# Funatiq/cuclark

Measured on AMD Instinct MI355X. Metric: Mreads/sec (10M x 150bp, k=31), higher is better.
Workload: dtype u64

## Files before the change

cuclark_amd/csrc/mic_kernels.hip:

```cpp
#include "mic_internal.h"
#include "mic_device.h"
#include "mic_ksketch.h"

#include <stdlib.h>

#ifndef MIC_EXP
#define MIC_EXP 0
#endif
#ifndef MIC_FUNNEL64
#define MIC_FUNNEL64 1
#endif
#ifndef MIC_X
#define MIC_X 0
#endif

namespace {

__device__ __forceinline__ uint4 load_slot_quarter(const uint4* p) {
  typedef unsigned int u4 __attribute__((ext_vector_type(4)));
  u4 t = __builtin_nontemporal_load((const u4*)p);
  return make_uint4(t.x, t.y, t.z, t.w);
}

__device__ __forceinline__ uint64_t kmer_from_dwords(uint32_t d0, uint32_t d1, uint32_t d2, int nt_in_dword, int k) {
  const int s = 2 * nt_in_dword;
  uint64_t a = ((uint64_t)d0 << 32) | d1;
#if MIC_FUNNEL64
  uint64_t x = (a << s) | ((uint64_t)d2 >> (32 - s));
#else
  uint64_t x = s ? ((a << s) | (uint64_t)(d2 >> (32 - s))) : a;
#endif
  return x >> (64 - 2 * k);
}


struct ReadAhead { uint32_t pp, pe, hdr, w; };

__device__ __forceinline__ void ahead_ptr(const MicQueryArgs& a, uint32_t r, ReadAhead& x) {
  if (r < a.n_reads) { x.pp = a.reads_ptr[r]; x.pe = a.reads_ptr[r + 1]; } else { x.pp = 0; x.pe = 0; }
}

__device__ __forceinline__ void ahead_window(const uint16_t* __restrict__ cont, uint32_t r, uint32_t n_reads, int lane,
                                             ReadAhead& x) {
  x.hdr = 0; x.w = 0;
  if (r < n_reads) {
    const uint32_t pp = __builtin_amdgcn_readfirstlane(x.pp);
    x.hdr = cont[pp];
    if (lane < 10) x.w = ((uint32_t)cont[pp + 1 + 2 * lane] << 16) | cont[pp + 2 + 2 * lane];
  }
}

__device__ __forceinline__ uint32_t window_word(const uint16_t* __restrict__ cont, uint32_t first, uint32_t cend,
                                                uint32_t base, int lane, bool use_ahead, const ReadAhead& x) {
  uint32_t w = 0;
  const uint32_t ci = first + base / 8 + 2 * lane;
  if (use_ahead) w = x.w;
  else if (lane < 10) w = ((ci < cend ? (uint32_t)cont[ci] : 0u) << 16) | (ci + 1 < cend ? (uint32_t)cont[ci + 1] : 0u);
  if (lane >= 10 || ci >= cend) w &= 0x0000FFFFu;
  if (lane >= 10 || ci + 1 >= cend) w &= 0xFFFF0000u;
  return w;
}

__device__ __forceinline__ uint32_t window_word_w(const uint16_t* __restrict__ cont, uint32_t first, uint32_t cend,
                                                  uint32_t base, int lane, bool use_ahead, uint32_t ahead_w) {
  uint32_t w = 0;
  const uint32_t ci = first + base / 8 + 2 * lane;
  if (use_ahead) w = ahead_w;
  else if (lane < 10) w = ((ci < cend ? (uint32_t)cont[ci] : 0u) << 16) | (ci + 1 < cend ? (uint32_t)cont[ci + 1] : 0u);
  if (lane >= 10 || ci >= cend) w &= 0x0000FFFFu;
  if (lane >= 10 || ci + 1 >= cend) w &= 0xFFFF0000u;
  return w;
}

struct Probe {
  uint32_t slot;
  uint32_t qlo, qhi;
};

template <bool KEY64>
__device__ __forceinline__ Probe make_probe(const MicTable& t, uint64_t kmer, bool active) {
  uint64_t c = canonical(kmer, t.k);
  uint64_t q = mic_div(c, t.div);
  uint64_t rem = c - q * t.div.d;
  Probe p;
  bool ok = active && rem >= t.shard_start && rem < t.shard_end;
  if (!KEY64) ok = ok && (q >> 32) == 0;
  p.slot = ok ? (uint32_t)(rem - t.shard_start) : 0xFFFFFFFFu;
// ... 245 lines not shown
  if (cover < w) step(w - cover);
}

__device__ __forceinline__ void sliding_min2(uint32_t& a0, uint32_t& a1, int w, int lane) {
  auto step = [&](int s) {
    const int src = (lane + s) & 63;
    const bool wrap = lane + s >= 64;
    uint32_t x0 = bperm(src, a0), x1 = bperm(src, a1);
    uint32_t n0 = wrap ? x1 : x0, n1 = wrap ? 0xFFFFFFFFu : x1;
    a0 = n0 < a0 ? n0 : a0; a1 = n1 < a1 ? n1 : a1;
  };
  int cover = 1;
  while (2 * cover <= w) { step(cover); cover *= 2; }
  if (cover < w) step(w - cover);
}

__device__ __forceinline__ uint32_t row_prefix_min(uint32_t t) {
  uint32_t x;
  x = (uint32_t)__builtin_amdgcn_update_dpp(-1, (int)t, 0x111, 0xF, 0xF, false); t = x < t ? x : t;
  x = (uint32_t)__builtin_amdgcn_update_dpp(-1, (int)t, 0x112, 0xF, 0xF, false); t = x < t ? x : t;
  x = (uint32_t)__builtin_amdgcn_update_dpp(-1, (int)t, 0x114, 0xF, 0xF, false); t = x < t ? x : t;
  x = (uint32_t)__builtin_amdgcn_update_dpp(-1, (int)t, 0x118, 0xF, 0xF, false); t = x < t ? x : t;
  return t;
}

__device__ __forceinline__ uint32_t row_suffix_min(uint32_t t) {
  uint32_t x;
  x = (uint32_t)__builtin_amdgcn_update_dpp(-1, (int)t, 0x101, 0xF, 0xF, false); t = x < t ? x : t;
  x = (uint32_t)__builtin_amdgcn_update_dpp(-1, (int)t, 0x102, 0xF, 0xF, false); t = x < t ? x : t;
  x = (uint32_t)__builtin_amdgcn_update_dpp(-1, (int)t, 0x104, 0xF, 0xF, false); t = x < t ? x : t;
  x = (uint32_t)__builtin_amdgcn_update_dpp(-1, (int)t, 0x108, 0xF, 0xF, false); t = x < t ? x : t;
  asm("" : "+v"(t));
  return t;
}

template <int BANKS>
__device__ __forceinline__ uint32_t with_row_in_front(uint32_t P) {
  const uint32_t f = (uint32_t)__builtin_amdgcn_update_dpp(-1, (int)P, 0x142, 0xE, BANKS, false);
  return f < P ? f : P;
}
__device__ __forceinline__ void sliding_min_rows(uint32_t& a0, uint32_t& a1, uint32_t a2, int W, int lane, int lane_inv) {
  const uint32_t P0 = row_prefix_min(a0), P1 = row_prefix_min(a1), P2 = row_prefix_min(a2);
  if (W > 16 && ((W - 16) & 3) == 0) {
    const uint32_t S0 = row_suffix_min(a0), S1 = row_suffix_min(a1);
    const int s = W - 16, bm = (1 << (s >> 2)) - 1;
    uint32_t Q0, Q1, Q2;
    switch (bm) {
      case 1: Q0 = with_row_in_front<1>(P0); Q1 = with_row_in_front<1>(P1); Q2 = with_row_in_front<1>(P2); break;
      case 3: Q0 = with_row_in_front<3>(P0); Q1 = with_row_in_front<3>(P1); Q2 = with_row_in_front<3>(P2); break;
      case 7: Q0 = with_row_in_front<7>(P0); Q1 = with_row_in_front<7>(P1); Q2 = with_row_in_front<7>(P2); break;
      default: Q0 = with_row_in_front<15>(P0); Q1 = with_row_in_front<15>(P1); Q2 = with_row_in_front<15>(P2); break;
    }
    const uint32_t f0 = __builtin_amdgcn_readlane(P0, 63), f1 = __builtin_amdgcn_readlane(P1, 63);
    const bool head = lane < s;
    const uint32_t h1 = f0 < Q1 ? f0 : Q1, h2 = f1 < Q2 ? f1 : Q2;
    Q1 = head ? h1 : Q1; Q2 = head ? h2 : Q2;
    const int at = (lane_inv << 2) + ((W - 1) << 2);
    const uint32_t z0 = (uint32_t)__builtin_amdgcn_ds_bpermute(at, (int)Q0), z1 = (uint32_t)__builtin_amdgcn_ds_bpermute(at, (int)Q1),
                   z2 = (uint32_t)__builtin_amdgcn_ds_bpermute(at, (int)Q2);
    const bool wz = lane >= 65 - W;
    const uint32_t v0 = wz ? z1 : z0, v1 = wz ? z2 : z1;
    a0 = v0 < S0 ? v0 : S0; a1 = v1 < S1 ? v1 : S1;
    return;
  }
  const uint32_t S0 = row_suffix_min(a0), S1 = row_suffix_min(a1), S2 = row_suffix_min(a2);
  const int at = lane_inv << 2;
  const uint32_t x0 = (uint32_t)__builtin_amdgcn_ds_bpermute(at + 60, (int)P0), x1 = (uint32_t)__builtin_amdgcn_ds_bpermute(at + 60, (int)P1),
                 x2 = (uint32_t)__builtin_amdgcn_ds_bpermute(at + 60, (int)P2);
  const bool wr = lane >= 49;
  const uint32_t n0 = wr ? x1 : x0, n1 = wr ? x2 : x1;
  uint32_t M0 = n0 < S0 ? n0 : S0, M1 = n1 < S1 ? n1 : S1;
  if (W > 16) {
    const uint32_t M2 = x2 < S2 ? x2 : S2;
    const int sh = (W - 16) << 2;
    const uint32_t y0 = (uint32_t)__builtin_amdgcn_ds_bpermute(at + sh, (int)M0), y1 = (uint32_t)__builtin_amdgcn_ds_bpermute(at + sh, (int)M1),
                   y2 = (uint32_t)__builtin_amdgcn_ds_bpermute(at + sh, (int)M2);
    const bool wy = lane >= 80 - W;
    const uint32_t v0 = wy ? y1 : y0, v1 = wy ? y2 : y1;
    M0 = v0 < M0 ? v0 : M0; M1 = v1 < M1 ? v1 : M1;
  }
  a0 = M0; a1 = M1;
}

template <bool CANON>
__device__ __forceinline__ void sampled_positions(uint32_t wd, int ln, int lane_inv, int k, int m, bool past, uint32_t& qa0, uint32_t& qa1) {
  const int w = k - m + 1, t = s_tlen(k, m), W = k - t + 1;
  const uint32_t pb = (uint32_t)lane_inv & 31u;
  uint32_t a0, a1, a2 = 0xFFFFFFFFu;
  if (t <= 16) {
    const int s1 = lane_inv - 1;
    const int ad = (s1 >> 4) << 2;
    const uint32_t tsh = 30u - 2u * (uint32_t)(s1 & 15);
    auto tkey = [&](int h) {
      const uint32_t W0 = (uint32_t)__builtin_amdgcn_ds_bpermute(ad + 16 * h, (int)wd), W1 = (uint32_t)__builtin_amdgcn_ds_bpermute(ad + 16 * h + 4, (int)wd);
      uint32_t tv = __builtin_amdgcn_alignbit(W0, W1, tsh) >> (32 - 2 * t);
      if (CANON) { const uint32_t tr = revcomp_bits32(tv, t); tv = tr < tv ? tr : tv; }
      return ((t <= 12 ? s_torder24(tv) : s_torder(tv)) & ~31u) | pb;
    };
    a0 = tkey(0); a1 = tkey(1);
    if (past) a2 = tkey(2);
  } else {
    auto tkey = [&](int h) {
      const int idx = 4 * h + (lane_inv >> 4);
      const uint32_t d0 = bperm(idx, wd), d1 = bperm(idx + 1, wd), d2 = bperm(idx + 2, wd);
      uint64_t tv = kmer_from_dwords(d0, d1, d2, lane_inv & 15, t);
      if (CANON) { const uint64_t tr = revcomp_bits(tv, t); tv = tr < tv ? tr : tv; }
      return (s_torder(tv) & ~31u) | pb;
    };
    a0 = tkey(0); a1 = tkey(1);
    if (past) a2 = tkey(2);
  }
  if (W >= 16) sliding_min_rows(a0, a1, a2, W, ln, lane_inv);
  else sliding_min3(a0, a1, a2, W, ln);
  uint32_t d0 = (a0 - pb) & 31u, d1 = (a1 - pb) & 31u;
  if (W == 2 * w) { const uint32_t e0 = d0 - (uint32_t)w, e1 = d1 - (uint32_t)w; d0 = e0 < d0 ? e0 : d0; d1 = e1 < d1 ? e1 : d1; }
  else if (W != w) {
    const uint32_t rcp = (1024u + (uint32_t)w - 1u) / (uint32_t)w;
    d0 -= (uint32_t)w * ((d0 * rcp) >> 10); d1 -= (uint32_t)w * ((d1 * rcp) >> 10);
  }
  qa0 = (uint32_t)lane_inv + d0; qa1 = 64u + (uint32_t)lane_inv + d1;
}

template <bool CANON>
__device__ __forceinline__ void sampled_positions3(uint32_t wd, int lane_inv, uint32_t n_act, uint32_t& p0, uint32_t& s0, uint32_t& s1, uint32_t& s2,
                                                    uint32_t& q0, uint32_t& q1, uint32_t& q2) {
  const int at = lane_inv << 2;
  const int ad = f3_dword(lane_inv) << 2;
  const uint32_t tsh = f3_shift(lane_inv);
  p0 = 3u * (uint32_t)lane_inv;
  const uint32_t np0 = 0u - p0;
  const uint32_t W0 = (uint32_t)__builtin_amdgcn_ds_bpermute(ad, (int)wd), W1 = (uint32_t)__builtin_amdgcn_ds_bpermute(ad + 4, (int)wd);
  const uint32_t X = __builtin_amdgcn_alignbit(W0, W1, tsh);
  uint32_t t0 = f3_tmer(X, 0), t1 = f3_tmer(X, 1), t2 = f3_tmer(X, 2);
  if (CANON) {
    const uint32_t br = __builtin_bitreverse32(X);
    const uint32_t Y = swap_comp_pairs(br >> 1, br << 1);
    t0 = f3_min(t0, f3_tmer_rc(Y, 0)); t1 = f3_min(t1, f3_tmer_rc(Y, 1)); t2 = f3_min(t2, f3_tmer_rc(Y, 2));
  }
  auto key = [](uint32_t tv, uint32_t pos) { return (uint32_t)__builtin_amdgcn_bitop3_b32(s_torder24(tv), pos, 31u, 0xD8); };
  const uint32_t k0 = key(t0, p0), k1 = key(t1, p0 + 1u), k2 = key(t2, p0 + 2u);
  const uint32_t T = f3_min3(k0, k1, k2), e12 = f3_min(k1, k2), e01 = f3_min(k0, k1);
  const uint32_t x1 = (uint32_t)__builtin_amdgcn_ds_bpermute(at + 4, (int)T);
  const uint32_t m2 = f3_min(T, x1);
  const uint32_t y = (uint32_t)__builtin_amdgcn_ds_bpermute(at + 8, (int)m2);
  const uint32_t m4 = f3_min(m2, y);
  const uint32_t z = (uint32_t)__builtin_amdgcn_ds_bpermute(at + 16, (int)m4);
  const uint32_t k0n = (uint32_t)__builtin_amdgcn_ds_bpermute(at + 32, (int)k0), e01n = (uint32_t)__builtin_amdgcn_ds_bpermute(at + 32, (int)e01);
  uint32_t r0, r1, r2;
  f3_combine(k2, e12, m4, x1, y, z, k0n, e01n, r0, r1, r2);
  auto sampled = [&](uint32_t r, uint32_t j) {
    const uint32_t d = (r + np0 - j) & 31u, e = d - (uint32_t)F3_WM;
    return f3_min(d, e) + p0 + j;
  };
  const int nv = (int)(n_act + np0);
  s0 = sampled(r0, 0u); s1 = sampled(r1, 1u); s2 = sampled(r2, 2u);
  q0 = nv > 0 ? s0 : ~0u; q1 = nv > 1 ? s1 : ~0u; q2 = nv > 2 ? s2 : ~0u;
}

#ifndef MIC_SPEC
#define MIC_SPEC 1
#endif
#ifndef MIC_M_WPB
#define MIC_M_WPB 4
#endif
template <int KK, int MM>
__global__ void __launch_bounds__(64 * MIC_M_WPB, 32 / MIC_M_WPB) query_kernel_m(const MicQueryArgs a) {
  __shared__ uint4 s_stage[MIC_M_WPB][MIC_RMAX * MIC_MSTRIDE + (MIC_RMAX / 8 - 1) * MIC_M_SKEW];
  __shared__ uint32_t s_run[MIC_M_WPB][MIC_RMAX];
  __shared__ uint32_t s_ahead[MIC_M_WPB][2][64];
  const int lane = threadIdx.x & 63;
  const int wv = __builtin_amdgcn_readfirstlane(threadIdx.x >> 6);
  uint4* stage = s_stage[wv];
  uint32_t* runslot = s_run[wv];
  const uint32_t wave0 = __builtin_amdgcn_readfirstlane(blockIdx.x * MIC_M_WPB + wv);
  const uint32_t n_waves = gridDim.x * MIC_M_WPB;
  const MicTable& t = a.t;
  const int k = KK ? KK : t.k, m = MM ? MM : t.m, w = k - m + 1;
  const uint4* __restrict__ slots = t.slots;
  const uint16_t* __restrict__ cont = a.cont;
  auto below = [](uint64_t mask) { return (uint32_t)__builtin_amdgcn_mbcnt_hi((uint32_t)(mask >> 32), __builtin_amdgcn_mbcnt_lo((uint32_t)mask, 0u)); };

  uint32_t* ahead0 = s_ahead[wv][0];
  uint32_t* ahead1 = s_ahead[wv][1];
  auto ahead_issue = [&](uint32_t* entry, uint32_t pp_w, uint32_t r_ptr) {
    const uint64_t abase = ((uint64_t)(cont + pp_w)) & ~3ULL;
    const uint32_t rr = r_ptr < a.n_reads ? r_ptr : a.n_reads - 1;
    const uint64_t pbase = (uint64_t)(a.reads_ptr + rr) - 48;
    uint32_t lv = (uint32_t)lane;
    asm volatile("" : "+v"(lv));
    const uint32_t li = lv < 14 ? lv : 0u;
    const uint64_t addr = (li < 12 ? abase : pbase) + 4 * li;
    __builtin_amdgcn_global_load_lds((const __attribute__((address_space(1))) void*)addr,
                                     (__attribute__((address_space(3))) void*)entry, 4, 0, 0);
  };
  auto ahead_take = [&](const uint32_t* entry, uint32_t pp_w, uint32_t& hdr, uint32_t& wword, uint32_t& npp, uint32_t& npe) {
    const uint32_t raw = entry[lane];
    npp = __builtin_amdgcn_readlane(raw, 12); npe = __builtin_amdgcn_readlane(raw, 13);
    const bool odd = (((uint64_t)(cont + pp_w)) >> 1) & 1;
    const uint32_t up = (uint32_t)__builtin_amdgcn_update_dpp(0, (int)raw, 0x101, 0xF, 0xF, true);
    const uint32_t first = __builtin_amdgcn_readfirstlane(raw);
    hdr = odd ? first >> 16 : first & 0xFFFFu;
    wword = odd ? ((up << 16) | (up >> 16)) : ((raw & 0xFFFF0000u) | (up & 0xFFFFu));
  };
  uint32_t cur_pp, cur_pe, cur_hdr, cur_w;
  uint32_t n_pp, n_pe;
  uint32_t ahead_sel;
  {
    const uint32_t r0 = wave0 < a.n_reads ? wave0 : a.n_reads - 1;
    cur_pp = __builtin_amdgcn_readfirstlane(a.reads_ptr[r0]); cur_pe = __builtin_amdgcn_readfirstlane(a.reads_ptr[r0 + 1]);
    ahead_issue(ahead0, cur_pp, wave0 + n_waves);
    asm volatile("s_waitcnt vmcnt(0)" ::: "memory");
    __builtin_amdgcn_wave_barrier();
    ahead_take(ahead0, cur_pp, cur_hdr, cur_w, n_pp, n_pe);
    ahead_issue(ahead1, n_pp, wave0 + 2 * n_waves);
    ahead_sel = 1;
  }
  for (uint32_t r = wave0; r < a.n_reads; r += n_waves) {
    uint32_t pp = cur_pp;
    const uint32_t pe = cur_pe;
    RowAcc acc; acc.label1 = 0; acc.count = 0;
    uint32_t n_ent = 0, overflow = 0, total = 0;
    bool first_part = true;

    while (pp < pe) {
      const uint32_t plen = __builtin_amdgcn_readfirstlane(first_part ? cur_hdr : (uint32_t)cont[pp]);
      const bool ahead_ok = first_part;
      first_part = false;
      if (plen == 0) break;
      const uint32_t first = pp + 1;
      pp = first + (plen + 7) / 8;
      if (plen < (uint32_t)k) continue;
      const uint32_t nk = plen - k + 1;
      const uint32_t cend = pp;
      for (uint32_t base = 0; base < nk; base += 128) {
        const uint32_t wd = window_word_w(cont, first, cend, base, lane, ahead_ok && base == 0, cur_w);
        uint64_t c[2]; bool act[2]; uint32_t hk0, hk1, hk2;
        const bool past = nk - base > (uint32_t)(129 - w);
        const bool tail_path = w <= 16;
        uint32_t tail = 0xFFFFFFFFu;
// ... 436 lines not shown
    const uint32_t l1 = __builtin_amdgcn_readlane(lab1, __builtin_ctzll(mm));
    const bool mine = lab1 == l1;
    mm &= ~wballot(mine);
    const uint32_t c = mine ? cnt : 0u;
    uint32_t sum = 0;
    {
      uint32_t v = c;
      v += (uint32_t)__builtin_amdgcn_update_dpp(0, (int)v, 0x111, 0xF, 0xF, true);
      v += (uint32_t)__builtin_amdgcn_update_dpp(0, (int)v, 0x112, 0xF, 0xF, true);
      v += (uint32_t)__builtin_amdgcn_update_dpp(0, (int)v, 0x114, 0xF, 0xF, true);
      v += (uint32_t)__builtin_amdgcn_update_dpp(0, (int)v, 0x118, 0xF, 0xF, true);
      sum = __builtin_amdgcn_readlane(v, 15) + __builtin_amdgcn_readlane(v, 31);
    }
    total += sum;
    row_add(acc, n_ent, overflow, l1, sum, lane);
  }
}

template <int KK, int MM, bool FWD, bool PART>
__global__ void __launch_bounds__(64 * MIC_M_WPB, 32 / MIC_M_WPB) query_kernel_r(const MicQueryArgs a) {
  __shared__ uint4 s_stage[MIC_M_WPB][MIC_RMAX * MIC_MSTRIDE + (MIC_RMAX / 8 - 1) * MIC_R_SKEW];
  __shared__ uint16_t s_rec[MIC_M_WPB][132];
  __shared__ uint32_t s_ahead[MIC_M_WPB][2][64];
  __shared__ uint32_t s_part[PART ? MIC_M_WPB : 1][2];
  const int lane = threadIdx.x & 63;
  const int wv = __builtin_amdgcn_readfirstlane(threadIdx.x >> 6);
  uint4* stage = s_stage[wv];
  uint16_t* rec = s_rec[wv];
  const uint32_t wave0 = __builtin_amdgcn_readfirstlane(blockIdx.x * MIC_M_WPB + wv);
  const uint32_t n_waves = gridDim.x * MIC_M_WPB;
  const MicTable& t = a.t;
  if (PART) { if (lane == 0) { s_part[wv][0] = t.slot_lo; s_part[wv][1] = t.slot_cnt; } __builtin_amdgcn_wave_barrier(); }
  const int k = KK ? KK : t.k, m = MM ? MM : t.m, ctx = k - m;
  const uint4* __restrict__ slots = t.slots;
  const uint16_t* __restrict__ cont = a.cont;
  auto below = [](uint64_t mask) { return (uint32_t)__builtin_amdgcn_mbcnt_hi((uint32_t)(mask >> 32), __builtin_amdgcn_mbcnt_lo((uint32_t)mask, 0u)); };

  uint32_t* ahead0 = s_ahead[wv][0];
  uint32_t* ahead1 = s_ahead[wv][1];
  auto ahead_issue = [&](uint32_t* entry, uint32_t pp_w, uint32_t r_ptr) {
    const uint64_t abase = ((uint64_t)(cont + pp_w)) & ~3ULL;
    const uint32_t rr = r_ptr < a.n_reads ? r_ptr : a.n_reads - 1;
    const uint64_t pbase = (uint64_t)(a.reads_ptr + rr) - 48;
    int ln = lane;
    asm volatile("" : "+v"(ln));
    if (ln < 12)
      __builtin_amdgcn_global_load_lds((const __attribute__((address_space(1))) void*)((const uint32_t*)abase + lane),
                                       (__attribute__((address_space(3))) void*)entry, 4, 0, 0);
    uint64_t pb = pbase + 48;
    asm volatile("" : "+s"(pb));
    if (ln < 2)
      __builtin_amdgcn_global_load_lds((const __attribute__((address_space(1))) void*)((const uint32_t*)pb + lane),
                                       (__attribute__((address_space(3))) void*)(entry + 12), 4, 0, 0);
  };
  auto ahead_take = [&](const uint32_t* entry, uint32_t pp_w, uint32_t& hdr, uint32_t& npp, uint32_t& npe) {
    const uint32_t raw = entry[lane];
    npp = __builtin_amdgcn_readlane(raw, 12); npe = __builtin_amdgcn_readlane(raw, 13);
    const bool odd = (((uint64_t)(cont + pp_w)) >> 1) & 1;
    const uint32_t first = __builtin_amdgcn_readfirstlane(raw);
    hdr = odd ? first >> 16 : first & 0xFFFFu;
  };
  auto ahead_word = [&](const uint32_t* entry, uint32_t pp_w) {
    const uint32_t raw = entry[lane];
    const bool odd = (((uint64_t)(cont + pp_w)) >> 1) & 1;
    const uint32_t up = (uint32_t)__builtin_amdgcn_update_dpp(0, (int)raw, 0x101, 0xF, 0xF, true);
    return __builtin_amdgcn_perm(up, raw, odd ? 0x05040706u : 0x03020504u);
  };
  uint32_t cur_pp, cur_pe, cur_hdr, n_pp, n_pe, ahead_sel;
  {
    const uint32_t r0 = wave0 < a.n_reads ? wave0 : a.n_reads - 1;
    cur_pp = __builtin_amdgcn_readfirstlane(a.reads_ptr[r0]); cur_pe = __builtin_amdgcn_readfirstlane(a.reads_ptr[r0 + 1]);
    ahead_issue(ahead0, cur_pp, wave0 + n_waves);
    asm volatile("s_waitcnt vmcnt(0)" ::: "memory");
    __builtin_amdgcn_wave_barrier();
    ahead_take(ahead0, cur_pp, cur_hdr, n_pp, n_pe);
    ahead_issue(ahead1, n_pp, wave0 + 2 * n_waves);
    ahead_sel = 1;
  }
  constexpr bool PIPE = KK != 0 && (MIC_R_PIPE >= 2 || (MIC_R_PIPE == 1 && FWD));
  struct Round {
    uint32_t G0, G1, G2, cur;
    int jmax, jmin, remaining;
  };
  auto front = [&](const uint32_t first, const uint32_t cend, const uint32_t base, const uint32_t nk, const bool use_ahead, uint32_t& wd_out) __attribute__((always_inline)) -> uint32_t {
    int ln = lane;
    asm volatile("" : "+v"(ln));
    const uint32_t wd = use_ahead ? ahead_word(ahead_sel ? ahead0 : ahead1, cur_pp)
                                  : window_word_w(cont, first, cend, base, ln, false, 0u);
    wd_out = wd;
    const uint32_t n_act = nk - base < 128u ? nk - base : 128u;
    if constexpr (KK == F3_K && MM == F3_M) {
      uint32_t p0, s0, s1, s2, q0, q1, q2;
      sampled_positions3<!FWD>(wd, lane, n_act, p0, s0, s1, s2, q0, q1, q2);
      const uint32_t pv = (uint32_t)__builtin_amdgcn_update_dpp(-1, (int)q2, 0x138, 0xF, 0xF, false);
      const bool f0 = q0 != pv, f1 = q1 != q0, f2 = q2 != q1;
      const uint64_t b0 = wballot(f0), b1 = wballot(f1), b2 = wballot(f2);
      const uint32_t R = __popcll(b0) + __popcll(b1) + __popcll(b2) - 1u;
      uint32_t c = __builtin_amdgcn_mbcnt_hi((uint32_t)(b0 >> 32), __builtin_amdgcn_mbcnt_lo((uint32_t)b0, 0u));
      c = __builtin_amdgcn_mbcnt_hi((uint32_t)(b1 >> 32), __builtin_amdgcn_mbcnt_lo((uint32_t)b1, c));
      c = __builtin_amdgcn_mbcnt_hi((uint32_t)(b2 >> 32), __builtin_amdgcn_mbcnt_lo((uint32_t)b2, c));
      __builtin_amdgcn_wave_barrier();
      const uint32_t c1 = c + (f0 ? 1u : 0u), c2 = c1 + (f1 ? 1u : 0u);
      if (f0) rec[c] = f3_record(s0, p0);
      if (f1) rec[c1] = f3_record(s1, p0 + 1u);
      if (f2) rec[c2] = f3_record(s2, p0 + 2u);
      __builtin_amdgcn_wave_barrier();
      return R;
    }
    const bool past = n_act + (uint32_t)(k - s_tlen(k, m)) >= 129u;
    uint32_t qa0, qa1;
    sampled_positions<!FWD>(wd, ln, lane, k, m, past, qa0, qa1);
    qa0 = (uint32_t)lane < n_act ? qa0 : 0xFFu;
    qa1 = 64u + (uint32_t)lane < n_act ? qa1 : 0xFFu;
    const uint32_t last0 = __builtin_amdgcn_readlane(qa0, 63);
    uint32_t p0 = (uint32_t)__builtin_amdgcn_update_dpp(-1, (int)qa0, 0x138, 0xF, 0xF, false);
    uint32_t p1 = (uint32_t)__builtin_amdgcn_update_dpp((int)last0, (int)qa1, 0x138, 0xF, 0xF, false);
    const bool f0 = qa0 != p0, f1 = qa1 != p1;
    const uint64_t b0 = wballot(f0), b1 = wballot(f1);
    const uint32_t R0 = __popcll(b0), R = R0 + __popcll(b1) - (n_act < 128u ? 1u : 0u);
    __builtin_amdgcn_wave_barrier();
    if (f0) rec[below(b0)] = (uint16_t)(qa0 | ((uint32_t)lane << 8));
    if (f1) rec[R0 + below(b1)] = (uint16_t)(qa1 | ((64u + (uint32_t)lane) << 8));
    if (__builtin_expect(n_act == 128u, 0)) {
      asm volatile("" ::: "memory");
      if (ln == 0) rec[R] = (uint16_t)(128u << 8);
    }
    __builtin_amdgcn_wave_barrier();
    return R;
  };
  const uint32_t xsh = (64u - 2u * (uint32_t)k) & 31u;
  auto region_x = [&](uint32_t A0, uint32_t A1, uint32_t& lo, uint32_t& hi) {
    if (k > 16) {
      lo = __builtin_amdgcn_alignbit(A0, A1, xsh) & (m >= 16 ? 0xFFFFFFFFu : (1u << ((2 * m) & 31)) - 1u);
      hi = m > 16 ? (A0 >> xsh) & ((1u << ((2 * m - 32) & 31)) - 1u) : 0u;
    } else {
      const uint64_t x = ((((uint64_t)A0 << 32) | A1) << (2 * ctx)) >> (64 - 2 * m);
      lo = (uint32_t)x; hi = (uint32_t)(x >> 32);
    }
  };
  auto setup = [&](const uint32_t wd, const uint32_t rbase, const uint32_t R, Round& L, uint32_t& nrun_out) __attribute__((always_inline)) {
    const uint32_t nrun = R - rbase < MIC_RMAX ? R - rbase : MIC_RMAX;
    nrun_out = nrun;
    const bool vr = (uint32_t)lane < nrun;
    const uint32_t ri = vr ? rbase + (uint32_t)lane : 0u;
    const uint32_t rc0 = rec[ri], rc1 = rec[ri + 1];
    const int qa = (int)(rc0 & 255u), i0 = (int)(rc0 >> 8);
    const int n = (int)(rc1 >> 8) - i0;
    const int s1 = qa - ctx - 1;
    const int D = s1 >> 4;
    const uint32_t tsh = 30u - 2u * (uint32_t)(s1 & 15);
    const int a0 = D << 2;
    const uint32_t W0 = (uint32_t)__builtin_amdgcn_ds_bpermute(a0, (int)wd), W1 = (uint32_t)__builtin_amdgcn_ds_bpermute(a0 + 4, (int)wd),
                   W2 = (uint32_t)__builtin_amdgcn_ds_bpermute(a0 + 8, (int)wd), W3 = (uint32_t)__builtin_amdgcn_ds_bpermute(a0 + 12, (int)wd);
    uint32_t G0 = __builtin_amdgcn_alignbit(W0, W1, tsh), G1 = __builtin_amdgcn_alignbit(W1, W2, tsh), G2 = __builtin_amdgcn_alignbit(W2, W3, tsh);
    uint32_t key, xhi;
    region_x(G0, G1, key, xhi);
    bool rev = false;
    if (!FWD) {
      const uint32_t sh = 96u - 2u * (uint32_t)(k + ctx);
      const uint32_t r0 = __builtin_bitreverse32(G2), r1 = __builtin_bitreverse32(G1), r2 = __builtin_bitreverse32(G0);
      uint32_t q0, q1, q2;
      if (KK != 0 && sh != 0) {
        q0 = swap_comp_pairs(__builtin_amdgcn_alignbit(r0, r1, 33u - sh), __builtin_amdgcn_alignbit(r0, r1, 31u - sh));
        q1 = swap_comp_pairs(__builtin_amdgcn_alignbit(r1, r2, 33u - sh), __builtin_amdgcn_alignbit(r1, r2, 31u - sh));
        q2 = swap_comp_pairs(r2 << (sh - 1u), r2 << (sh + 1u));
      } else {
        q0 = sh ? __builtin_amdgcn_alignbit(r0, r1, 32u - sh) : r0;
        q1 = sh ? __builtin_amdgcn_alignbit(r1, r2, 32u - sh) : r1;
        q2 = r2 << sh;
        q0 = swap_comp_pairs(q0 >> 1, q0 << 1); q1 = swap_comp_pairs(q1 >> 1, q1 << 1); q2 = swap_comp_pairs(q2 >> 1, q2 << 1);
      }
      uint32_t kr, hr;
      region_x(q0, q1, kr, hr);
      rev = hr < xhi || (hr == xhi && kr < key);
      G0 = rev ? q0 : G0; G1 = rev ? q1 : G1; G2 = rev ? q2 : G2;
      key = rev ? kr : key; xhi = rev ? hr : xhi;
    }
    const int jmaxf = qa - i0, jminf = jmaxf - n + 1;
    const int jmax = rev ? ctx - jminf : jmaxf, jmin = rev ? ctx - jmaxf : jminf;
    uint32_t cur = vr ? sslot_of_x32(key, xhi, (uint32_t)t.n_main) : 0xFFFFFFFFu;
    bool mine = vr;
    if (PART) {
      mine = vr && cur - s_part[wv][0] < s_part[wv][1];
      cur = mine ? cur : 0xFFFFFFFFu;
    }
    L.G0 = G0; L.G1 = G1; L.G2 = G2; L.cur = cur;
    L.jmax = jmax; L.jmin = jmin; L.remaining = mine ? n : 0;
  };
  auto issue = [&](const uint32_t cur, const uint32_t nrun) __attribute__((always_inline)) {
    uint32_t sidx[MIC_RMAX / 8];
    int ln = lane;
    asm volatile("" : "+v"(ln));
    __builtin_amdgcn_wave_barrier();
    if (ln < MIC_RMAX) ((uint32_t*)stage)[lane] = cur;
    __builtin_amdgcn_wave_barrier();
    uint32_t so = (uint32_t)(uintptr_t)(__attribute__((address_space(3))) void*)stage;
    asm volatile("" : "+s"(so));
#pragma unroll
    for (int i = 0; i < MIC_RMAX / 8; ++i) sidx[i] = ((const uint32_t*)stage)[8 * i + (lane >> 3)];
#pragma unroll
    for (int i = 0; i < MIC_RMAX / 8; ++i) {
      if (8u * i >= nrun) break;
      if (sidx[i] != 0xFFFFFFFFu)
        __builtin_amdgcn_global_load_lds((const __attribute__((address_space(1))) void*)(slots + (uint64_t)sidx[i] * 8 + (lane & 7)),
                                         (__attribute__((address_space(3))) void*)(uintptr_t)(so + 16u * (64 + MIC_R_SKEW) * (uint32_t)i), 16, 0, 0);
    }
  };
  auto consume = [&](Round& L, RowAcc& acc, uint32_t& n_ent, uint32_t& overflow, uint32_t& total, uint32_t& cg) __attribute__((always_inline)) {
    const uint32_t G0 = L.G0, G1 = L.G1, G2 = L.G2;
    uint32_t key, xhi_;
    region_x(G0, G1, key, xhi_);
    const int jmax = L.jmax, jmin = L.jmin;
    uint32_t cur = L.cur;
    int remaining = L.remaining;
    bool again = false;
    do {
      if (again) issue(cur, MIC_RMAX);
      again = true;
      asm volatile("s_waitcnt vmcnt(0)" ::: "memory");
      __builtin_amdgcn_wave_barrier();
      const bool vl = cur != 0xFFFFFFFFu;
      const uint32_t* q = (const uint32_t*)(stage + (vl ? staged_at((uint32_t)lane) : 0));
      const uint4 ka = *(const uint4*)q;
      const uint2 kb = *(const uint2*)(q + 4);
      uint32_t e = (ka.x < key) + (ka.y < key) + (ka.z < key) + (ka.w < key) + (kb.x < key) + (kb.y < key);
      const uint32_t mz = q[30];
      bool more = vl && e < 6;
      e = e < 5 ? e : 5;
      for (;;) {
// ... 17 lines not shown
#if !(MIC_X & 1)
        remaining = (same && mineq && (pl >> 16) == 0) ? MIC_R_CROWDED : remaining;
#endif
        const uint32_t lab_new = (pl & 0xFFFFu) + 1u;
        tally_counts(hits ? lab_new : 0u, hits, acc, n_ent, overflow, total, lane);
        remaining -= (int)hits;
        more = same && remaining > 0 && e < 5;
        e += more ? 1u : 0u;
        if (!wballot(more)) break;
      }
      const bool nx = vl && remaining > 0 && (mz & MIC_S_NEXT);
      cur = 0xFFFFFFFFu;
      if (wballot(nx)) { if (nx && q[5] <= key) cur = q[31]; }
    } while (wballot(cur != 0xFFFFFFFFu));
    if (!(MIC_X & 2) && __builtin_expect(wballot(remaining <= MIC_R_CROWDED) != 0, 0)) {
      const bool crowded = remaining <= MIC_R_CROWDED;
      const uint32_t n_c = (uint32_t)__popcll(wballot(crowded));
      uint64_t kpv = (uint64_t)__builtin_amdgcn_kernarg_segment_ptr();
      asm volatile("" : "+v"(kpv));
      const MicQueryArgs* kv = (const MicQueryArgs*)kpv;
      uint32_t* cw = kv->crowd;
      uint32_t* itb = kv->crowd_items;
      const uint32_t icap = kv->crowd_item_cap;
      uint32_t ib = 0xFFFFFFFFu;
      if (cw != nullptr && cg != MIC_CG_DENSE) {
        uint32_t v = 0;
        if (lane == 0) v = atomicAdd(&cw[1], n_c);
        ib = __builtin_amdgcn_readfirstlane(v);
      }
      asm volatile("" : "+v"(ib));
      const bool room = ib <= icap && n_c <= icap - ib;
      if (crowded && room) {
        uint32_t* it = itb + 8 * ((size_t)ib + below(wballot(crowded)));
        it[0] = G0; it[1] = G1; it[2] = G2; it[3] = (uint32_t)jmin | ((uint32_t)jmax << 8);
        it[4] = cg;
      }
      cg = __builtin_amdgcn_readfirstlane(room ? (ib | ((n_c - 1u) << 27)) : MIC_CG_DENSE);
    }
  };
  auto finish = [&](const RowAcc& acc, uint32_t n_ent, uint32_t total, uint32_t overflow, uint32_t r, const uint32_t cg) __attribute__((always_inline)) {
    uint32_t spilled = 0;
    if (!(MIC_X & 4) && __builtin_expect(cg != MIC_CG_NONE, 0)) {
      uint64_t kpv = (uint64_t)__builtin_amdgcn_kernarg_segment_ptr();
      asm volatile("" : "+v"(kpv));
      const MicQueryArgs* kv = (const MicQueryArgs*)kpv;
      uint32_t* cw = kv->crowd;
      uint32_t* pool = kv->crowd_pool;
      const uint32_t pcap = kv->crowd_pend_cap, wcap = kv->crowd_pool_cap;
      uint32_t p = 0xFFFFFFFFu, off = 0;
      if (cg != MIC_CG_DENSE) {
        if (lane == 0) { p = atomicAdd(&cw[0], 1u); off = atomicAdd(&cw[2], 2u * n_ent); }
        p = __builtin_amdgcn_readfirstlane(p); off = __builtin_amdgcn_readfirstlane(off);
      }
      asm volatile("" : "+v"(p), "+v"(off));
      const bool room = off <= wcap && 2u * n_ent <= wcap - off;
      if (p < pcap) {
        uint32_t* pd = cw + MIC_CROWD_HDR + 8 * (size_t)p;
        if (lane == 0) { pd[0] = r; pd[1] = total; pd[2] = room ? (n_ent | (overflow << 8)) : 0xFFFFFFFFu; pd[3] = off; pd[4] = cg; }
        if (room && (uint32_t)lane < n_ent) { uint32_t* pe_ = pool + (size_t)off + 2 * lane; pe_[0] = acc.label1; pe_[1] = acc.count; }
      }
      spilled = __builtin_amdgcn_readfirstlane((p < pcap && room) ? 1u : 0u);
      if (!spilled) {
        if (lane == 0 && cw != nullptr && cg != MIC_CG_DENSE) atomicAdd(&cw[3], 1u);
        overflow = 1;
      }
    }
    if (!spilled) {
      uint64_t kp = (uint64_t)__builtin_amdgcn_kernarg_segment_ptr();
      asm volatile("" : "+s"(kp));
      const __attribute__((address_space(4))) MicQueryArgs* kc = (const __attribute__((address_space(4))) MicQueryArgs*)kp;
      struct { uint32_t* results; uint32_t* rows; uint32_t* flagged; uint32_t row_words, flagged_cap; } fa;
      fa.results = kc->results; fa.rows = kc->rows; fa.flagged = kc->flagged; fa.row_words = kc->row_words; fa.flagged_cap = kc->flagged_cap;
      finish_read(acc, n_ent, total, overflow, r, fa, lane);
    }
  };

  uint32_t r = wave0; bool p_valid = false;
  auto step = [&](Round& P, Round& N) __attribute__((always_inline)) -> bool {
    const bool have = r < a.n_reads;
    uint32_t pp = cur_pp;
    const uint32_t pe = cur_pe;
    bool shape = false, simple = false;
    uint32_t n_nrun = 0, plen0 = 0, pp1 = 0;
    if (have) {
      plen0 = cur_hdr; pp1 = pp + 1 + (plen0 + 7) / 8;
      shape = plen0 - (uint32_t)k < 128u && pp1 == pe;
      if (!shape && plen0 - (uint32_t)k < 128u && pp1 < pe) {
        const uint32_t rel = pp1 - cur_pp + (uint32_t)((((uint64_t)(cont + cur_pp)) >> 1) & 1);
        if (rel < 24u) {
          const uint32_t v = (ahead_sel ? ahead0 : ahead1)[rel >> 1];
          shape = __builtin_amdgcn_readfirstlane((rel & 1u) ? v >> 16 : v & 0xFFFFu) == 0;
        }
      }
      if (PIPE && shape) {
        uint32_t n_wd;
        const uint32_t R = front(pp + 1, pp1, 0u, plen0 - (uint32_t)k + 1u, true, n_wd);
        if (R <= MIC_RMAX) { setup(n_wd, 0u, R, N, n_nrun); simple = true; }
      }
    }
    if (PIPE && p_valid) {
      RowAcc acc; acc.label1 = 0; acc.count = 0;
      uint32_t n_ent = 0, overflow = 0, total = 0, cg = MIC_CG_NONE;
      consume(P, acc, n_ent, overflow, total, cg);
      finish(acc, n_ent, total, overflow, r - n_waves, cg);
    } else {
      asm volatile("s_waitcnt vmcnt(0)" ::: "memory");
    }
    if (!have) return false;
    if (!simple) {
      RowAcc acc; acc.label1 = 0; acc.count = 0;
      uint32_t n_ent = 0, overflow = 0, total = 0, cg = MIC_CG_NONE;
      auto chunk = [&](const uint32_t first, const uint32_t cend, const uint32_t base, const uint32_t nk, const bool use_ahead) __attribute__((always_inline)) {
        uint32_t wd;
        const uint32_t R = front(first, cend, base, nk, use_ahead, wd);
        for (uint32_t rbase = 0; rbase < R; rbase += MIC_RMAX) {
          Round L; uint32_t nrun;
          setup(wd, rbase, R, L, nrun);
          issue(L.cur, nrun);
          consume(L, acc, n_ent, overflow, total, cg);
        }
      };
      if (!PIPE && shape) chunk(pp + 1, pp1, 0u, plen0 - (uint32_t)k + 1u, true);
      else {
        bool first_part = true;
        while (pp < pe) {
          uint32_t plen;
          {
            const uint32_t rel = pp - cur_pp + (uint32_t)((((uint64_t)(cont + cur_pp)) >> 1) & 1);
            if (first_part) plen = cur_hdr;
            else if (rel < 24u) {
              const uint32_t v = (ahead_sel ? ahead0 : ahead1)[rel >> 1];
              plen = __builtin_amdgcn_readfirstlane((rel & 1u) ? v >> 16 : v & 0xFFFFu);
            } else plen = __builtin_amdgcn_readfirstlane((uint32_t)cont[pp]);
          }
          const bool ahead_ok = first_part;
          first_part = false;
          if (plen == 0) break;
          const uint32_t first = pp + 1;
          pp = first + (plen + 7) / 8;
          if (plen < (uint32_t)k) continue;
          const uint32_t nk = plen - k + 1;
          const uint32_t cend = pp;
          for (uint32_t base = 0; base < nk; base += 128) chunk(first, cend, base, nk, ahead_ok && base == 0);
        }
      }
      finish(acc, n_ent, total, overflow, r, cg);
    }
    uint32_t t_hdr, t_pp, t_pe;
    __builtin_amdgcn_wave_barrier();
    ahead_take(ahead_sel ? ahead1 : ahead0, n_pp, t_hdr, t_pp, t_pe);
    __builtin_amdgcn_wave_barrier();
    ahead_issue(ahead_sel ? ahead0 : ahead1, t_pp, r + 3 * n_waves);
    ahead_sel ^= 1;
    cur_pp = n_pp; cur_pe = n_pe; cur_hdr = t_hdr; n_pp = t_pp; n_pe = t_pe;
    p_valid = simple;
    if (simple) issue(N.cur, n_nrun);
    r += n_waves;
    return true;
  };
  Round Ra, Rb;
  while (step(Ra, Rb) && step(Rb, Ra)) {}
}

__global__ void __launch_bounds__(256) crowd_finish_kernel(const MicQueryArgs a) {
  const int lane = threadIdx.x & 63;
  const uint32_t wave0 = __builtin_amdgcn_readfirstlane(blockIdx.x * 4 + (threadIdx.x >> 6)), n_waves = gridDim.x * 4;
  const uint32_t* __restrict__ cw = a.crowd;
  const uint32_t pcap = a.crowd_pend_cap;
  uint32_t np = cw[0];
  np = np < pcap ? np : pcap;
  const uint32_t* __restrict__ pend = cw + MIC_CROWD_HDR;
  const uint32_t* __restrict__ items = a.crowd_items;
  const uint32_t* __restrict__ pool = a.crowd_pool;
  const uint4* __restrict__ side = a.t.side;
  const uint32_t smask = a.t.side_mask;
  const int k = a.t.k, ctx = k - a.t.m;
  for (uint32_t p = wave0; p < np; p += n_waves) {
    const uint4 h = *(const uint4*)(pend + 8 * (size_t)p);
    const uint32_t r = __builtin_amdgcn_readfirstlane(h.x), meta = __builtin_amdgcn_readfirstlane(h.z), off = __builtin_amdgcn_readfirstlane(h.w);
    uint32_t total = __builtin_amdgcn_readfirstlane(h.y);
    uint32_t g = __builtin_amdgcn_readfirstlane(pend[8 * (size_t)p + 4]);
    if (meta == 0xFFFFFFFFu) continue;
    uint32_t n_ent = meta & 0xFFu, overflow = (meta >> 8) & 1u;
    RowAcc acc; acc.label1 = 0; acc.count = 0;
    if ((uint32_t)lane < n_ent) { const uint2 e = *(const uint2*)(pool + off + 2 * lane); acc.label1 = e.x; acc.count = e.y; }
    while (g != MIC_CG_NONE) {
      const uint32_t ib = g & 0x7FFFFFFu, n_c = (g >> 27) + 1u;
      g = __builtin_amdgcn_readfirstlane(items[8 * (size_t)ib + 4]);
      for (uint32_t b = 0; b < n_c; b += 4) {
        const uint32_t idx = b + ((uint32_t)lane >> 4);
        const bool valid = idx < n_c;
        uint4 it = make_uint4(0, 0, 0, 0);
        if (valid) it = *(const uint4*)(items + 8 * (size_t)(ib + idx));
        const int jmin = (int)(it.w & 0xFFu), jmax = (int)((it.w >> 8) & 0xFFu);
        int j = jmin + (lane & 15);
        bool go = valid && j <= jmax;
        j = go ? j : jmin;
        const uint64_t K = s_extract(it.x, it.y, it.z, ctx - j, k);
        uint32_t hsh = s_side_hash(K, smask), got = 0;
        while (wballot(go)) {
// ... 479 lines not shown
```

Baseline: 2120.

## Pipeline two-part reads by joining both parts into one gapped window

Reads made of two short parts (for example, sequences split by an N) used to drop off the pipelined single-window fast path into the slower chunked loop. A new join helper checks that both parts fit within the prefetched header entry and builds one combined window. Minimizer positions and k-mer validity are computed with a gap offset so that k-mers spanning the part boundary are masked out. This adds extra shape checks and template variants on the hot path, which raises code size and register pressure, to benefit whatever fraction of reads has this two-part layout.

```diff
diff --git a/cuclark_amd/csrc/mic_join2.h b/cuclark_amd/csrc/mic_join2.h
--- /dev/null
+++ b/cuclark_amd/csrc/mic_join2.h
@@ -0,0 +1,78 @@
+#ifndef MIC_JOIN2_H
+#define MIC_JOIN2_H
+
+#include <stdint.h>
+
+#if defined(__HIPCC__)
+#define J2_FN __host__ __device__ __forceinline__
+#else
+#define J2_FN static inline
+#endif
+
+#define J2_ENTRY_U16 24
+#define J2_CHUNK 128
+
+struct J2Shape {
+  uint32_t ok;
+  uint32_t len1, len2;
+  uint32_t b2;
+  uint32_t n_act;
+  uint32_t g0, g1;
+};
+
+J2_FN uint32_t j2_half(uint32_t dword, uint32_t u) { return (u & 1u) ? dword >> 16 : dword & 0xFFFFu; }
+
+#define J2_NONE 0xFFFFFFFFu
+J2_FN uint32_t j2_slot2(uint32_t plen0, uint32_t span, uint32_t odd, uint32_t k) {
+  if (plen0 - k >= (uint32_t)J2_CHUNK) return J2_NONE;
+  const uint32_t h2 = 1u + (plen0 + 7u) / 8u;
+  return h2 < span && h2 + odd < (uint32_t)J2_ENTRY_U16 ? h2 + odd : J2_NONE;
+}
+template <typename At>
+J2_FN J2Shape j2_shape(uint32_t plen0, uint32_t slot2, uint32_t span, uint32_t odd, uint32_t k, At&& at) {
+  J2Shape s;
+  s.ok = 0; s.len1 = plen0; s.len2 = 0; s.b2 = 0; s.n_act = 0; s.g0 = 0; s.g1 = 0;
+  if (j2_slot2(plen0, span, odd, k) == J2_NONE) return s;
+  const uint32_t h2 = 1u + (plen0 + 7u) / 8u;
+  const uint32_t len2 = slot2;
+  if (len2 - k >= (uint32_t)J2_CHUNK) return s;
+  const uint32_t end = h2 + 1u + (len2 + 7u) / 8u;
+  if (end + odd > (uint32_t)J2_ENTRY_U16 || end > span) return s;
+  if (end < span) {
+    if (end + odd >= (uint32_t)J2_ENTRY_U16) return s;
+    if (at(end + odd) != 0u) return s;
+  }
+  const uint32_t n_act = plen0 + len2 - k + 1u;
+  if (n_act > (uint32_t)J2_CHUNK) return s;
+  s.ok = 1; s.len2 = len2; s.b2 = h2 + 1u + odd; s.n_act = n_act; s.g0 = plen0 - k + 1u; s.g1 = plen0;
+  return s;
+}
+
+J2_FN int j2_t(uint32_t j, uint32_t len1) { const int t = 16 * (int)j - (int)len1; return t < -16 ? -16 : t; }
+J2_FN uint32_t j2_nt(uint32_t j, uint32_t len1, uint32_t b2) { return (uint32_t)(8 * (int)b2 + j2_t(j, len1)); }
+J2_FN uint32_t j2_dword(uint32_t j, uint32_t len1, uint32_t b2) { return j2_nt(j, len1, b2) >> 4; }
+J2_FN uint32_t j2_window(uint32_t w1, uint32_t d0, uint32_t d1, uint32_t j, uint32_t len1, uint32_t b2) {
+  const uint64_t z = ((uint64_t)((d0 << 16) | (d0 >> 16)) << 32) | ((d1 << 16) | (d1 >> 16));
+  const uint32_t p = (uint32_t)((z << (2u * (j2_nt(j, len1, b2) & 15u))) >> 32);
+  const int r = -j2_t(j, len1);
+  const uint32_t m = (uint32_t)(0xFFFFFFFFull >> (2 * (r < 0 ? 0 : r)));
+  return (w1 & ~m) | (p & m);
+}
+
+J2_FN uint32_t j2_part_offset(uint32_t last, uint32_t len1) { return last >= len1 ? len1 : 0u; }
+J2_FN bool j2_is_kmer(uint32_t pos, uint32_t n_act, uint32_t g0, uint32_t k) { return pos < n_act && pos - g0 >= k - 1u; }
+
+#if !defined(__HIP_DEVICE_COMPILE__)
+static inline uint32_t j2_model_w1(const uint32_t entry[64], uint32_t odd, uint32_t j) {
+  const uint32_t raw = entry[j & 63u], up = entry[(j + 1u) & 63u];
+  return odd ? (up << 16) | (up >> 16) : (raw & 0xFFFF0000u) | (up & 0xFFFFu);
+}
+static inline void j2_model(const uint32_t entry[64], uint32_t odd, const J2Shape& s, uint32_t wd[12]) {
+  for (uint32_t j = 0; j < 12; ++j) {
+    const uint32_t d = j2_dword(j, s.len1, s.b2);
+    wd[j] = j2_window(j2_model_w1(entry, odd, j), entry[d & 63u], entry[(d + 1u) & 63u], j, s.len1, s.b2);
+  }
+}
+#endif
+
+#endif
diff --git a/cuclark_amd/csrc/mic_kernels.hip b/cuclark_amd/csrc/mic_kernels.hip
--- a/cuclark_amd/csrc/mic_kernels.hip
+++ b/cuclark_amd/csrc/mic_kernels.hip
@@ -1,8 +1,10 @@
 #include "mic_internal.h"
 #include "mic_device.h"
 #include "mic_ksketch.h"
+#include "mic_join2.h"
 
 #include <stdlib.h>
+#include <type_traits>
 
 #ifndef MIC_EXP
 #define MIC_EXP 0
@@ -414,10 +416,15 @@
   a0 = M0; a1 = M1;
 }
 
-template <bool CANON>
-__device__ __forceinline__ void sampled_positions(uint32_t wd, int ln, int lane_inv, int k, int m, bool past, uint32_t& qa0, uint32_t& qa1) {
+template <bool CANON, bool GAP = false>
+__device__ __forceinline__ void sampled_positions(uint32_t wd, int ln, int lane_inv, int k, int m, bool past, uint32_t& qa0, uint32_t& qa1,
+                                                  uint32_t len1 = 0) {
   const int w = k - m + 1, t = s_tlen(k, m), W = k - t + 1;
-  const uint32_t pb = (uint32_t)lane_inv & 31u;
+  const uint32_t pb0 = (uint32_t)lane_inv & 31u;
+  auto pb_of = [&](int h) {
+    const uint32_t pos = 64u * (uint32_t)h + (uint32_t)lane_inv;
+    return GAP ? (pos - j2_part_offset(pos, len1)) & 31u : pb0;
+  };
   uint32_t a0, a1, a2 = 0xFFFFFFFFu;
   if (t <= 16) {
     const int s1 = lane_inv - 1;
@@ -427,7 +434,7 @@
       const uint32_t W0 = (uint32_t)__builtin_amdgcn_ds_bpermute(ad + 16 * h, (int)wd), W1 = (uint32_t)__builtin_amdgcn_ds_bpermute(ad + 16 * h + 4, (int)wd);
       uint32_t tv = __builtin_amdgcn_alignbit(W0, W1, tsh) >> (32 - 2 * t);
       if (CANON) { const uint32_t tr = revcomp_bits32(tv, t); tv = tr < tv ? tr : tv; }
-      return ((t <= 12 ? s_torder24(tv) : s_torder(tv)) & ~31u) | pb;
+      return ((t <= 12 ? s_torder24(tv) : s_torder(tv)) & ~31u) | pb_of(h);
     };
     a0 = tkey(0); a1 = tkey(1);
     if (past) a2 = tkey(2);
@@ -437,14 +444,14 @@
       const uint32_t d0 = bperm(idx, wd), d1 = bperm(idx + 1, wd), d2 = bperm(idx + 2, wd);
       uint64_t tv = kmer_from_dwords(d0, d1, d2, lane_inv & 15, t);
       if (CANON) { const uint64_t tr = revcomp_bits(tv, t); tv = tr < tv ? tr : tv; }
-      return (s_torder(tv) & ~31u) | pb;
+      return (s_torder(tv) & ~31u) | pb_of(h);
     };
     a0 = tkey(0); a1 = tkey(1);
     if (past) a2 = tkey(2);
   }
   if (W >= 16) sliding_min_rows(a0, a1, a2, W, ln, lane_inv);
   else sliding_min3(a0, a1, a2, W, ln);
-  uint32_t d0 = (a0 - pb) & 31u, d1 = (a1 - pb) & 31u;
+  uint32_t d0 = (a0 - pb_of(0)) & 31u, d1 = (a1 - pb_of(1)) & 31u;
   if (W == 2 * w) { const uint32_t e0 = d0 - (uint32_t)w, e1 = d1 - (uint32_t)w; d0 = e0 < d0 ? e0 : d0; d1 = e1 < d1 ? e1 : d1; }
   else if (W != w) {
     const uint32_t rcp = (1024u + (uint32_t)w - 1u) / (uint32_t)w;
@@ -453,14 +460,15 @@
   qa0 = (uint32_t)lane_inv + d0; qa1 = 64u + (uint32_t)lane_inv + d1;
 }
 
-template <bool CANON>
+template <bool CANON, bool GAP = false>
 __device__ __forceinline__ void sampled_positions3(uint32_t wd, int lane_inv, uint32_t n_act, uint32_t& p0, uint32_t& s0, uint32_t& s1, uint32_t& s2,
-                                                    uint32_t& q0, uint32_t& q1, uint32_t& q2) {
+                                                    uint32_t& q0, uint32_t& q1, uint32_t& q2, uint32_t len1 = 0, uint32_t g0 = 0) {
   const int at = lane_inv << 2;
   const int ad = f3_dword(lane_inv) << 2;
   const uint32_t tsh = f3_shift(lane_inv);
   p0 = 3u * (uint32_t)lane_inv;
-  const uint32_t np0 = 0u - p0;
+  const uint32_t pk = GAP ? p0 - j2_part_offset(p0 + 2u, len1) : p0;
+  const uint32_t np0 = 0u - pk;
   const uint32_t W0 = (uint32_t)__builtin_amdgcn_ds_bpermute(ad, (int)wd), W1 = (uint32_t)__builtin_amdgcn_ds_bpermute(ad + 4, (int)wd);
   const uint32_t X = __builtin_amdgcn_alignbit(W0, W1, tsh);
   uint32_t t0 = f3_tmer(X, 0), t1 = f3_tmer(X, 1), t2 = f3_tmer(X, 2);
@@ -470,7 +478,7 @@
     t0 = f3_min(t0, f3_tmer_rc(Y, 0)); t1 = f3_min(t1, f3_tmer_rc(Y, 1)); t2 = f3_min(t2, f3_tmer_rc(Y, 2));
   }
   auto key = [](uint32_t tv, uint32_t pos) { return (uint32_t)__builtin_amdgcn_bitop3_b32(s_torder24(tv), pos, 31u, 0xD8); };
-  const uint32_t k0 = key(t0, p0), k1 = key(t1, p0 + 1u), k2 = key(t2, p0 + 2u);
+  const uint32_t k0 = key(t0, pk), k1 = key(t1, pk + 1u), k2 = key(t2, pk + 2u);
   const uint32_t T = f3_min3(k0, k1, k2), e12 = f3_min(k1, k2), e01 = f3_min(k0, k1);
   const uint32_t x1 = (uint32_t)__builtin_amdgcn_ds_bpermute(at + 4, (int)T);
   const uint32_t m2 = f3_min(T, x1);
@@ -484,9 +492,13 @@
     const uint32_t d = (r + np0 - j) & 31u, e = d - (uint32_t)F3_WM;
     return f3_min(d, e) + p0 + j;
   };
-  const int nv = (int)(n_act + np0);
+  const int nv = GAP ? (int)(n_act - p0) : (int)(n_act + np0);
   s0 = sampled(r0, 0u); s1 = sampled(r1, 1u); s2 = sampled(r2, 2u);
   q0 = nv > 0 ? s0 : ~0u; q1 = nv > 1 ? s1 : ~0u; q2 = nv > 2 ? s2 : ~0u;
+  if (GAP) {
+    const uint32_t gv = p0 - g0;
+    q0 = gv >= (uint32_t)(F3_K - 1) ? q0 : ~0u; q1 = gv + 1u >= (uint32_t)(F3_K - 1) ? q1 : ~0u; q2 = gv + 2u >= (uint32_t)(F3_K - 1) ? q2 : ~0u;
+  }
 }
 
 #ifndef MIC_SPEC
@@ -1089,16 +1101,29 @@
     uint32_t G0, G1, G2, cur;
     int jmax, jmin, remaining;
   };
-  auto front = [&](const uint32_t first, const uint32_t cend, const uint32_t base, const uint32_t nk, const bool use_ahead, uint32_t& wd_out) __attribute__((always_inline)) -> uint32_t {
+  struct NoGap {};
+  struct Gap { uint32_t len1, b2, g0; };
+  auto front = [&](const uint32_t first, const uint32_t cend, const uint32_t base, const uint32_t nk, const bool use_ahead, uint32_t& wd_out,
+                   const auto gp) __attribute__((always_inline)) -> uint32_t {
+    constexpr bool GAP = std::is_same<decltype(gp), const Gap>::value;
     int ln = lane;
     asm volatile("" : "+v"(ln));
-    const uint32_t wd = use_ahead ? ahead_word(ahead_sel ? ahead0 : ahead1, cur_pp)
-                                  : window_word_w(cont, first, cend, base, ln, false, 0u);
+    uint32_t wd;
+    if constexpr (GAP) {
+      const uint32_t* entry = ahead_sel ? ahead0 : ahead1;
+      const uint32_t j = (uint32_t)ln < 12u ? (uint32_t)ln : 0u;
+      const uint32_t d = j2_dword(j, gp.len1, gp.b2);
+      wd = j2_window(ahead_word(entry, cur_pp), entry[d], entry[d + 1u], j, gp.len1, gp.b2);
+    } else {
+      wd = use_ahead ? ahead_word(ahead_sel ? ahead0 : ahead1, cur_pp)
+                     : window_word_w(cont, first, cend, base, ln, false, 0u);
+    }
     wd_out = wd;
     const uint32_t n_act = nk - base < 128u ? nk - base : 128u;
     if constexpr (KK == F3_K && MM == F3_M) {
       uint32_t p0, s0, s1, s2, q0, q1, q2;
-      sampled_positions3<!FWD>(wd, lane, n_act, p0, s0, s1, s2, q0, q1, q2);
+      if constexpr (GAP) sampled_positions3<!FWD, true>(wd, lane, n_act, p0, s0, s1, s2, q0, q1, q2, gp.len1, gp.g0);
+      else sampled_positions3<!FWD>(wd, lane, n_act, p0, s0, s1, s2, q0, q1, q2);
       const uint32_t pv = (uint32_t)__builtin_amdgcn_update_dpp(-1, (int)q2, 0x138, 0xF, 0xF, false);
       const bool f0 = q0 != pv, f1 = q1 != q0, f2 = q2 != q1;
       const uint64_t b0 = wballot(f0), b1 = wballot(f1), b2 = wballot(f2);
@@ -1116,9 +1141,14 @@
     }
     const bool past = n_act + (uint32_t)(k - s_tlen(k, m)) >= 129u;
     uint32_t qa0, qa1;
-    sampled_positions<!FWD>(wd, ln, lane, k, m, past, qa0, qa1);
+    if constexpr (GAP) sampled_positions<!FWD, true>(wd, ln, lane, k, m, past, qa0, qa1, gp.len1);
+    else sampled_positions<!FWD>(wd, ln, lane, k, m, past, qa0, qa1);
     qa0 = (uint32_t)lane < n_act ? qa0 : 0xFFu;
     qa1 = 64u + (uint32_t)lane < n_act ? qa1 : 0xFFu;
+    if constexpr (GAP) {
+      qa0 = (uint32_t)lane - gp.g0 >= (uint32_t)(k - 1) ? qa0 : 0xFFu;
+      qa1 = 64u + (uint32_t)lane - gp.g0 >= (uint32_t)(k - 1) ? qa1 : 0xFFu;
+    }
     const uint32_t last0 = __builtin_amdgcn_readlane(qa0, 63);
     uint32_t p0 = (uint32_t)__builtin_amdgcn_update_dpp(-1, (int)qa0, 0x138, 0xF, 0xF, false);
     uint32_t p1 = (uint32_t)__builtin_amdgcn_update_dpp((int)last0, (int)qa1, 0x138, 0xF, 0xF, false);
@@ -1145,13 +1175,15 @@
       lo = (uint32_t)x; hi = (uint32_t)(x >> 32);
     }
   };
-  auto setup = [&](const uint32_t wd, const uint32_t rbase, const uint32_t R, Round& L, uint32_t& nrun_out) __attribute__((always_inline)) {
+  auto setup = [&](const uint32_t wd, const uint32_t rbase, const uint32_t R, Round& L, uint32_t& nrun_out, const auto gp) __attribute__((always_inline)) {
+    constexpr bool GAP = std::is_same<decltype(gp), const Gap>::value;
     const uint32_t nrun = R - rbase < MIC_RMAX ? R - rbase : MIC_RMAX;
     nrun_out = nrun;
-    const bool vr = (uint32_t)lane < nrun;
+    bool vr = (uint32_t)lane < nrun;
     const uint32_t ri = vr ? rbase + (uint32_t)lane : 0u;
     const uint32_t rc0 = rec[ri], rc1 = rec[ri + 1];
     const int qa = (int)(rc0 & 255u), i0 = (int)(rc0 >> 8);
+    if constexpr (GAP) vr = vr && (uint32_t)i0 != gp.g0;
     const int n = (int)(rc1 >> 8) - i0;
     const int s1 = qa - ctx - 1;
     const int D = s1 >> 4;
@@ -1335,6 +1367,7 @@
     const uint32_t pe = cur_pe;
     bool shape = false, simple = false;
     uint32_t n_nrun = 0, plen0 = 0, pp1 = 0;
+    uint32_t slot2 = J2_NONE;
     if (have) {
       plen0 = cur_hdr; pp1 = pp + 1 + (plen0 + 7) / 8;
       shape = plen0 - (uint32_t)k < 128u && pp1 == pe;
@@ -1342,14 +1375,24 @@
         const uint32_t rel = pp1 - cur_pp + (uint32_t)((((uint64_t)(cont + cur_pp)) >> 1) & 1);
         if (rel < 24u) {
           const uint32_t v = (ahead_sel ? ahead0 : ahead1)[rel >> 1];
-          shape = __builtin_amdgcn_readfirstlane((rel & 1u) ? v >> 16 : v & 0xFFFFu) == 0;
+          slot2 = __builtin_amdgcn_readfirstlane((rel & 1u) ? v >> 16 : v & 0xFFFFu);
+          shape = slot2 == 0;
         }
       }
+      uint32_t n_wd = 0, R = MIC_RMAX + 1u, g0 = 0xFFFFFFFFu;
       if (PIPE && shape) {
-        uint32_t n_wd;
-        const uint32_t R = front(pp + 1, pp1, 0u, plen0 - (uint32_t)k + 1u, true, n_wd);
-        if (R <= MIC_RMAX) { setup(n_wd, 0u, R, N, n_nrun); simple = true; }
+        R = front(pp + 1, pp1, 0u, plen0 - (uint32_t)k + 1u, true, n_wd, NoGap{});
+      } else if constexpr (PIPE) {
+        const uint32_t odd = (uint32_t)((((uint64_t)(cont + cur_pp)) >> 1) & 1);
+        const uint32_t* entry = ahead_sel ? ahead0 : ahead1;
+        const J2Shape j2 = j2_shape(plen0, slot2, pe - pp, odd, (uint32_t)k,
+                                    [&](uint32_t u) { return (uint32_t)__builtin_amdgcn_readfirstlane(j2_half(entry[u >> 1], u)); });
+        if (__builtin_expect(j2.ok != 0u, 0)) {
+          R = front(pp + 1, pp1, 0u, j2.n_act, true, n_wd, Gap{j2.len1, j2.b2, j2.g0});
+          g0 = j2.g0;
+        }
       }
+      if (PIPE && R <= MIC_RMAX) { setup(n_wd, 0u, R, N, n_nrun, Gap{0u, 0u, g0}); simple = true; }
     }
     if (PIPE && p_valid) {
       RowAcc acc; acc.label1 = 0; acc.count = 0;
@@ -1365,10 +1408,10 @@
       uint32_t n_ent = 0, overflow = 0, total = 0, cg = MIC_CG_NONE;
       auto chunk = [&](const uint32_t first, const uint32_t cend, const uint32_t base, const uint32_t nk, const bool use_ahead) __attribute__((always_inline)) {
         uint32_t wd;
-        const uint32_t R = front(first, cend, base, nk, use_ahead, wd);
+        const uint32_t R = front(first, cend, base, nk, use_ahead, wd, NoGap{});
         for (uint32_t rbase = 0; rbase < R; rbase += MIC_RMAX) {
           Round L; uint32_t nrun;
-          setup(wd, rbase, R, L, nrun);
+          setup(wd, rbase, R, L, nrun, NoGap{});
           issue(L.cur, nrun);
           consume(L, acc, n_ent, overflow, total, cg);
         }
```

After: 2219, median of 6. 1.05x the previous value.
